# wenhao728/VORTA

Measured on AMD Instinct MI355X. Metric: video_tokens_per_sec (routed-attention denoising step, HunyuanVideo 720p 129f), higher is better.
Workload: dtype fp16

## Files before the change

### include/vorta_hip.h

```cpp
#ifndef VORTA_HIP_H
#define VORTA_HIP_H

#include <stdint.h>

#ifdef __cplusplus
extern "C" {
#endif

#define VORTA_OK 0
#define VORTA_EINVAL (-1)
#define VORTA_EUNSUPPORTED (-2)
#define VORTA_ELAUNCH (-3)

#define VORTA_ABI_VERSION 9

typedef enum vorta_dtype {
  VORTA_BF16 = 0,
  VORTA_FP16 = 1,
  VORTA_FP32 = 2,
  VORTA_FP8E4M3 = 3,
  VORTA_INT8 = 4
} vorta_dtype;

typedef struct vorta_tensor {
// ... 117 lines not shown
  float* k_bias;
  int64_t k_bias_stride_h;
  float* q_prep;
  float* k_head_scale;
  float* ws;
  int32_t flags;
  int32_t seg_len;
  int32_t tail_first;
  int32_t tail_len;
  int32_t slot_first;
  int32_t slot_count;
} vorta_i8_quant_args;

int vorta_i8_quantize_k(const vorta_i8_quant_args* args, void* hip_stream);

int vorta_i8_tail_flags(const vorta_tensor* k8, int32_t heads, int32_t n_tokens, const int32_t* row_map, float min_rms, int32_t* flags,
                        void* hip_stream);
int vorta_split_heads(const int32_t* head_list, const int32_t* n_heads_dev, int32_t n_heads, const int32_t* flags,
                      int32_t* list0, int32_t* list1, int32_t* counts, void* hip_stream);

typedef struct vorta_attn_i8_ext {
  uint32_t struct_size;
  int32_t flags;
  const float* k_bias;
  int64_t k_bias_stride_h;
  const float* q_prep;
  int64_t q_prep_stride_h;
  const float* k_head_scale;
  const float* v_descale;
  int64_t v_descale_stride_h;
// ... 141 lines not shown
```

### vorta_amd/_C.py

```python
import ctypes as C
import os

_HERE = os.path.dirname(os.path.abspath(__file__))
LIB_PATH = os.environ.get("VORTA_HIP_LIB") or os.path.join(_HERE, "csrc", "libvorta_hip.so")

VORTA_OK, VORTA_EINVAL, VORTA_EUNSUPPORTED, VORTA_ELAUNCH = 0, -1, -2, -3
VORTA_BF16, VORTA_FP16, VORTA_FP32, VORTA_FP8E4M3, VORTA_INT8 = 0, 1, 2, 3, 4
ABI_VERSION = 9

_i32, _i64, _u32, _f32, _vp = C.c_int32, C.c_int64, C.c_uint32, C.c_float, C.c_void_p


class Tensor(C.Structure):
    _fields_ = [("ptr", _vp), ("stride_h", _i64), ("stride_s", _i64)]


class AttnArgs(C.Structure):
    _fields_ = [
        ("struct_size", _u32), ("dtype", _i32), ("head_dim", _i32), ("n_heads", _i32),
        ("q", Tensor), ("k", Tensor), ("v", Tensor), ("o", Tensor),
        ("head_list", _vp), ("n_heads_dev", _vp),
        ("n_q", _i32), ("q_group_len", _i32), ("q_row_offset", _i32), ("q_valid", _i32),
        ("q_rows", _vp), ("q_rows_stride_h", _i64),
        ("n_kv", _i32), ("kv_row_offset", _i32),
# ... 136 lines not shown
NORM_ROPE_BWD_PARTS = 1024

SYMBOLS = {
    "vorta_attn_fwd": (C.c_int, [C.POINTER(AttnArgs), _vp]),
    "vorta_attn_fwd_batch": (C.c_int, [C.POINTER(AttnArgs), _i32, _vp]),
    "vorta_attn_plan": (C.c_int, [C.POINTER(AttnArgs), C.POINTER(_i32), C.POINTER(_i64), C.POINTER(_i32)]),
    "vorta_attn_workspace_bytes": (C.c_int, [C.POINTER(AttnArgs), C.POINTER(C.c_uint64), C.POINTER(C.c_uint64)]),
    "vorta_fp8_quant_ws_floats": (C.c_int, [_i32, _i32]),
    "vorta_fp8_quant_ws_partials": (C.c_int, [_i32, _i32, C.POINTER(_i64), C.POINTER(_i64)]),
    "vorta_fp8_quantize_qkv": (C.c_int, [C.POINTER(Fp8QuantArgs), _vp]),
    "vorta_fp8_v_absmax": (C.c_int, [C.POINTER(Fp8VArgs), _vp]),
    "vorta_fp8_v_convert": (C.c_int, [C.POINTER(Fp8VArgs), _vp]),
    "vorta_attn_fwd_fp8": (C.c_int, [C.POINTER(AttnArgs), C.POINTER(AttnFp8Ext), _vp]),
    "vorta_attn_fwd_batch_fp8": (C.c_int, [C.POINTER(AttnArgs), C.POINTER(AttnFp8Ext), _i32, _vp]),
    "vorta_i8_quantize_k": (C.c_int, [C.POINTER(I8QuantArgs), _vp]),
    "vorta_i8_tail_flags": (C.c_int, [C.POINTER(Tensor), _i32, _i32, _vp, C.c_float, _vp, _vp]),
    "vorta_split_heads": (C.c_int, [_vp, _vp, _i32, _vp, _vp, _vp, _vp, _vp]),
    "vorta_attn_fwd_i8": (C.c_int, [C.POINTER(AttnArgs), C.POINTER(AttnI8Ext), _vp]),
    "vorta_attn_fwd_batch_i8": (C.c_int, [C.POINTER(AttnArgs), C.POINTER(AttnI8Ext), _i32, _vp]),
    "vorta_coreset_select": (C.c_int, [C.POINTER(CoresetArgs), _vp]),
    "vorta_sta_table_sizes": (C.c_int, [C.POINTER(StaArgs), C.POINTER(_i32), C.POINTER(_i32), C.POINTER(_i32)]),
    "vorta_sta_build_tables": (C.c_int, [C.POINTER(StaArgs), _vp]),
    "vorta_router_route": (C.c_int, [C.POINTER(RouterArgs), _vp]),
    "vorta_route_scores": (C.c_int, [C.POINTER(RouterArgs), _vp]),
    "vorta_route_plan": (C.c_int, [C.POINTER(RouterArgs), C.c_int32, _vp]),
    "vorta_qk_norm_rope": (C.c_int, [C.POINTER(NormRopeArgs), _vp]),
    "vorta_qk_norm_rope_bwd": (C.c_int, [C.POINTER(NormRopeBwdArgs), _vp]),
    "vorta_mix_experts": (C.c_int, [C.POINTER(MixArgs), _vp]),
    "vorta_attn_bwd": (C.c_int, [C.POINTER(AttnBwdArgs), _vp]),
    "vorta_mix_experts_bwd": (C.c_int, [C.POINTER(MixBwdArgs), _vp]),
# ... 59 lines not shown
```

### vorta_amd/build.py

```python
import os
import subprocess
import sys

HERE = os.path.dirname(os.path.abspath(__file__))
CSRC = os.path.join(HERE, "csrc")
INCLUDE = os.path.join(os.path.dirname(HERE), "include")
LIB = os.path.join(CSRC, "libvorta_hip.so")
SOURCES = ["api.hip", "attn_fwd.hip", "attn_bwd.hip", "attn_fwd_fp8.hip", "attn_fwd_mx.hip", "attn_fwd_i8.hip", "fp8_quant.hip", "i8_quant.hip", "coreset.hip",
           "sta_tables.hip", "router.hip", "qk_norm_rope.hip", "qk_norm_rope_bwd.hip", "mix.hip", "permute.hip"]
FLAGS = ["--offload-arch=gfx950", "-O3", "-std=c++17", "-fPIC", "-fno-slp-vectorize", "-mllvm", "-enable-post-misched=0",
         "-I" + INCLUDE, "-I" + CSRC, "-Wno-unused-result"]


def _newer(src, dst):
    return (not os.path.exists(dst)) or os.path.getmtime(src) > os.path.getmtime(dst)


def build(force: bool = False, verbose: bool = True, extra_flags=None, suffix: str = "") -> str:
    hipcc = os.environ.get("HIPCC", "/opt/rocm/bin/hipcc")
    extra = list(extra_flags) if extra_flags is not None else os.environ.get("VORTA_EXTRA_FLAGS", "").split()
    suffix = suffix or os.environ.get("VORTA_BUILD_SUFFIX", "")
    if extra and not suffix:
        raise SystemExit("VORTA_EXTRA_FLAGS needs VORTA_BUILD_SUFFIX: experimental flags are never built into "
                         "libvorta_hip.so itself")
    lib = LIB if not suffix else os.path.join(CSRC, f"libvorta_hip{suffix}.so")
    deps = [os.path.join(CSRC, "common.h"), os.path.join(CSRC, "attn_common.h"), os.path.join(CSRC, "attn_fwd_fp8_diag.inc"),
            os.path.join(CSRC, "attn_fwd_i8_diag.inc"), os.path.join(CSRC, "attn_fwd_diag.inc"), os.path.join(INCLUDE, "vorta_hip.h")]
    if extra:
        extra = extra + ['-DVORTA_VARIANT_FLAGS="%s"' % " ".join(extra).replace('"', "'")]
    objs = []
    for s in SOURCES:
        src = os.path.join(CSRC, s)
        obj = os.path.join(CSRC, s.replace(".hip", f"{suffix}.o"))
        if force or _newer(src, obj) or any(_newer(d, obj) for d in deps):
            cmd = [hipcc] + FLAGS + extra + ["-c", src, "-o", obj]
            if verbose:
                print("[vorta_amd.build]", " ".join(cmd), flush=True)
            subprocess.check_call(cmd)
        objs.append(obj)
    if force or any(_newer(o, lib) for o in objs):
        cmd = [hipcc, "--offload-arch=gfx950", "-shared", "-fPIC", "-o", lib] + objs
        if verbose:
# ... 43 lines not shown
```

### vorta_amd/csrc/fp8_quant.hip

```cpp
#include <hip/hip_runtime.h>
#include <stdint.h>

#include "vorta_hip.h"
#include "common.h"

namespace {

constexpr int D = 128;
constexpr float V_TARGET = 240.f;
constexpr float E4M3_MAX = 448.f;
constexpr int MEAN_SAMPLES = 1024;
constexpr int SAMPLE_CHUNKS = 8;
constexpr int MEAN_BLOCKS = SAMPLE_CHUNKS + 1;

struct QParams {
  const char* x[3]; int64_t x_sh[3], x_ss[3];
  char* y[3]; int64_t y_sh[3], y_ss[3];
  int heads, n_tokens, rows_per_block;
  int seg_len, chunks_per_seg;
  int tail_first, tail_len;
  int mean_stride, mean_cand;
  int64_t video_tokens;
  int64_t total_tokens;
  int64_t token_offset;
  const int32_t* src_map;
// ... 201 lines not shown
  if (p.n_which < 3) return;
  float mv = p.ws[2 * H + h * D + d];
  if (p.v_per_head) {
    red[d] = mv;
    __syncthreads();
    for (int s = 64; s > 0; s >>= 1) {
      if (d < s) red[d] = fmaxf(red[d], red[d + s]);
      __syncthreads();
    }
    mv = red[0];
  }
  vmul[h * D + d] = mv > 0.f ? V_TARGET / mv : 0.f;
  p.v_descale[h * D + d] = mv / V_TARGET;
}

__device__ __forceinline__ float clamp448(float x) { return __builtin_amdgcn_fmed3f(x, -E4M3_MAX, E4M3_MAX); }

template <typename T>
__global__ __launch_bounds__(256) void fp8_convert_kernel(const QParams p) {
  typedef __attribute__((ext_vector_type(8))) T T8;
  const int which = blockIdx.z, H = p.heads;
  int r0, r1, h, hphys;
  block_rows(p, r0, r1, h, hphys);
  if (r0 >= r1) return;
  const int t = threadIdx.x, cc = t & 7, rl = t >> 3;
  const int hout = hphys;
  if (p.src_map && p.seg_len <= 0) {
    const int hs = p.src_map[hout];
    if (hs < 0) return;
    h = hphys = hs;
  }
// ... 164 lines not shown
    if (e != hipSuccess) return vorta_set_hip_error(e);
  }
  hipLaunchKernelGGL(fp8_scales_kernel, dim3((unsigned)hn), dim3(128), 0, st, p);
  e = hipGetLastError();
  if (e != hipSuccess) return vorta_set_hip_error(e);
  grid.z = (unsigned)n_which;
  if (bf) hipLaunchKernelGGL((fp8_convert_kernel<__bf16>), grid, dim3(256), 0, st, p);
  else hipLaunchKernelGGL((fp8_convert_kernel<_Float16>), grid, dim3(256), 0, st, p);
  e = hipGetLastError();
  if (e != hipSuccess) return vorta_set_hip_error(e);
  return VORTA_OK;
}

namespace {

struct VParams {
  const char* x; int64_t x_sh, x_ss;
  char* y; int64_t y_sh, y_ss;
  int heads, n_tokens, rows_per_block, per_head;
  const int32_t* src_map;
  float* amax; float* v_descale;
};

template <typename T>
__global__ __launch_bounds__(256) void fp8_v_absmax_kernel(const VParams p) {
  typedef __attribute__((ext_vector_type(8))) T T8;
  const int h = blockIdx.y;
  const int r0 = blockIdx.x * p.rows_per_block, r1 = min(r0 + p.rows_per_block, p.n_tokens);
  const int t = threadIdx.x, cc = t & 15, rl = t >> 4;
  const char* base = p.x + (int64_t)h * p.x_sh + cc * 16;
  float m[8];
#pragma unroll
  for (int i = 0; i < 8; ++i) m[i] = 0.f;
  for (int r = r0 + rl; r < r1; r += 16) {
    const T8 v = *(const T8*)(base + (int64_t)r * p.x_ss);
#pragma unroll
    for (int i = 0; i < 8; ++i) m[i] = fmaxf(m[i], fabsf(to_f(v[i])));
  }
  __shared__ float red[16][D + 1];
#pragma unroll
  for (int i = 0; i < 8; ++i) red[rl][cc * 8 + i] = m[i];
  __syncthreads();
  if (t < D) {
    float cm = 0.f;
#pragma unroll
    for (int j = 0; j < 16; ++j) cm = fmaxf(cm, red[j][t]);
    atomicMax((unsigned*)p.amax + h * D + t, __float_as_uint(cm));
  }
}

template <typename T>
__global__ __launch_bounds__(256) void fp8_v_convert_kernel(const VParams p) {
  typedef __attribute__((ext_vector_type(8))) T T8;
  const int h = blockIdx.y, hs = p.src_map ? p.src_map[h] : h;
  const int r0 = blockIdx.x * p.rows_per_block, r1 = min(r0 + p.rows_per_block, p.n_tokens);
  const int t = threadIdx.x, cc = t & 7, rl = t >> 3;
  float mul[16];
  float ph = 0.f;
  if (p.per_head) {
    for (int d = 0; d < D; ++d) ph = fmaxf(ph, p.amax[hs * D + d]);
  }
#pragma unroll
  for (int i = 0; i < 16; ++i) {
    const float mv = p.per_head ? ph : p.amax[hs * D + cc * 16 + i];
    mul[i] = mv > 0.f ? V_TARGET / mv : 0.f;
  }
  if (p.v_descale && blockIdx.x == 0 && t < D) {
    const float mv = p.per_head ? ph : p.amax[hs * D + t];
    p.v_descale[h * D + t] = mv / V_TARGET;
  }
  const char* src = p.x + (int64_t)hs * p.x_sh + cc * 32;
  char* dst = p.y + (int64_t)h * p.y_sh + cc * 16;
  for (int r = r0 + rl; r < r1; r += 32) {
    const T8 a = *(const T8*)(src + (int64_t)r * p.x_ss);
    const T8 b = *(const T8*)(src + (int64_t)r * p.x_ss + 16);
    float f[16];
#pragma unroll
    for (int i = 0; i < 8; ++i) {
      f[i] = clamp448(to_f(a[i]) * mul[i]);
      f[8 + i] = clamp448(to_f(b[i]) * mul[8 + i]);
    }
    u32x4 o;
#pragma unroll
    for (int w = 0; w < 4; ++w) {
      int lo = __builtin_amdgcn_cvt_pk_fp8_f32(f[4 * w], f[4 * w + 1], 0, false);
      o[w] = (uint32_t)__builtin_amdgcn_cvt_pk_fp8_f32(f[4 * w + 2], f[4 * w + 3], lo, true);
    }
    *(u32x4*)(dst + (int64_t)r * p.y_ss) = o;
  }
}

int v_params(const vorta_fp8_v_args* a, bool convert, VParams& p) {
  if (!a || a->struct_size != sizeof(vorta_fp8_v_args)) return VORTA_EINVAL;
  if (a->dtype != VORTA_BF16 && a->dtype != VORTA_FP16) return VORTA_EUNSUPPORTED;
  if (a->head_dim != D) return VORTA_EUNSUPPORTED;
  if (a->heads < 0 || a->n_tokens < 0) return VORTA_EINVAL;
  if (a->heads == 0 || a->n_tokens == 0) return 1;
  if (!a->amax || !a->v.ptr || ((uintptr_t)a->v.ptr & 15) || (a->v.stride_s % 8) || (a->v.stride_h % 8) || a->v.stride_s < D)
    return VORTA_EINVAL;
  p.x = (const char*)a->v.ptr; p.x_sh = a->v.stride_h * 2; p.x_ss = a->v.stride_s * 2;
  if (convert) {
    if (!a->v8.ptr || ((uintptr_t)a->v8.ptr & 15) || (a->v8.stride_s % 16) || (a->v8.stride_h % 16) || a->v8.stride_s < D)
      return VORTA_EINVAL;
    p.y = (char*)a->v8.ptr; p.y_sh = a->v8.stride_h; p.y_ss = a->v8.stride_s;
  }
  p.heads = a->heads; p.n_tokens = a->n_tokens;
  p.rows_per_block = 1024;
  p.per_head = a->flags & 1;
  p.src_map = convert ? a->src_map : nullptr;
  p.amax = a->amax; p.v_descale = convert ? a->v_descale : nullptr;
  return VORTA_OK;
}

}

extern "C" int vorta_fp8_v_absmax(const vorta_fp8_v_args* a, void* hip_stream) {
  VParams p{};
  const int rc = v_params(a, false, p);
  if (rc) return rc < 0 ? rc : VORTA_OK;
  const dim3 grid((unsigned)((p.n_tokens + p.rows_per_block - 1) / p.rows_per_block), (unsigned)p.heads);
  hipStream_t st = (hipStream_t)hip_stream;
  if (a->dtype == VORTA_BF16) hipLaunchKernelGGL((fp8_v_absmax_kernel<__bf16>), grid, dim3(256), 0, st, p);
  else hipLaunchKernelGGL((fp8_v_absmax_kernel<_Float16>), grid, dim3(256), 0, st, p);
  const hipError_t e = hipGetLastError();
  return e == hipSuccess ? VORTA_OK : vorta_set_hip_error(e);
}
// ... 13 lines not shown
```

### vorta_amd/csrc/i8_quant.hip

```cpp
#include <hip/hip_runtime.h>
#include <stdint.h>

#include "vorta_hip.h"
#include "common.h"

namespace {

constexpr int D = 128;
constexpr int SAMPLES = 1024;

struct IParams {
  const char* q; const char* k; int64_t q_sh, q_ss, k_sh, k_ss;
  char* k8; int64_t k8_sh, k8_ss;
  float* k_bias; int64_t k_bias_sh;
  float* q_prep; float* k_head_scale; float* ws;
  int heads, n_tokens, rows_per_block;
  int seg_len, chunks_per_seg, tail_first, tail_len;
  int slot_first, slot_count;
  int64_t video_tokens, total_tokens;
  int stride, cand;
  int no_smooth, no_center;
};

template <typename T>
__global__ __launch_bounds__(1024) void i8_stats_kernel(const IParams p) {
#pragma clang fp contract(off)
  typedef __attribute__((ext_vector_type(8))) T T8;
  const int h = p.slot_first + blockIdx.x;
  const int t = threadIdx.x, cg = t & 15, rl = t >> 4;
  auto row_of = [&](int64_t tok) -> int64_t {
    if (p.seg_len <= 0) return tok;
    if (tok < p.video_tokens) return ((tok / p.seg_len) * p.heads + h) * p.seg_len + tok % p.seg_len;
    return (int64_t)p.tail_first + (int64_t)h * p.seg_len + (tok - p.video_tokens);
  };
  const char* kb = p.k + (p.seg_len > 0 ? 0 : (int64_t)h * p.k_sh) + cg * 16;
  const char* qb = p.q + (p.seg_len > 0 ? 0 : (int64_t)h * p.q_sh) + cg * 16;
// ... 39 lines not shown
    const float var_k = mk2 - mean_k * mean_k;
    const float mean_q = red[2][0][t] / n;
    const float mq2 = red[3][0][t] / n;
    const float var_q = mq2 - mean_q * mean_q;
    float s = 1.f;
    if (!p.no_smooth && var_k > 0.f && var_q > 0.f) {
      s = sqrtf(sqrtf(var_k / var_q));
      s = fminf(fmaxf(s, 0.125f), 8.f);
    }
    p.ws[h * D + t] = p.no_center ? 0.f : mean_k;
    p.ws[(p.heads + h) * D + t] = 1.f / s;
    p.q_prep[(2 * h) * D + t] = p.no_center ? 0.f : mean_q;
    p.q_prep[(2 * h + 1) * D + t] = s;
  }
  if (t == 0) ((int*)p.ws)[2 * p.heads * D + h] = 0;
}

__device__ __forceinline__ void block_rows(const IParams& p, int& r0, int& r1, int& head, int& hphys) {
  if (p.seg_len > 0) {
    const int per = p.slot_count * p.chunks_per_seg;
    const int sg = blockIdx.x / per, rem = blockIdx.x - sg * per;
    const int si = rem / p.chunks_per_seg, c = rem - si * p.chunks_per_seg;
    const int seg = sg * p.heads + p.slot_first + si;
    const int s0 = seg * p.seg_len;
    r0 = s0 + c * p.rows_per_block;
    const int seg_rows = s0 >= p.tail_first ? p.tail_len : p.seg_len;
    r1 = min(min(r0 + p.rows_per_block, s0 + seg_rows), p.n_tokens);
    head = seg % p.heads;
    hphys = 0;
  } else {
    head = hphys = blockIdx.y;
    r0 = blockIdx.x * p.rows_per_block;
    r1 = min(r0 + p.rows_per_block, p.n_tokens);
  }
}

template <typename T, int PASS>
__global__ __launch_bounds__(256) void i8_rows_kernel(const IParams p) {
#pragma clang fp contract(off)
  typedef __attribute__((ext_vector_type(8))) T T8;
  int r0, r1, h, hphys;
  block_rows(p, r0, r1, h, hphys);
  if (r0 >= r1) return;
  const int t = threadIdx.x, cg = t & 15, rl = t >> 4;
  float c[8], is[8], cq[8];
#pragma unroll
  for (int e = 0; e < 8; ++e) {
    c[e] = p.ws[h * D + cg * 8 + e];
    is[e] = p.ws[(p.heads + h) * D + cg * 8 + e];
    cq[e] = p.q_prep[(2 * h) * D + cg * 8 + e];
  }
  const char* src = p.k + (int64_t)hphys * p.k_sh + cg * 16;
  char* dst = p.k8 + (int64_t)hphys * p.k8_sh + cg * 8;
  float* bias = p.k_bias + (int64_t)hphys * p.k_bias_sh;
  const float am_head = PASS == 1 ? __int_as_float(((const int*)p.ws)[2 * p.heads * D + h]) : 0.f;
  const float inv = am_head > 0.f ? 127.f / am_head : 0.f;
  float am = 0.f;
// ... 31 lines not shown
          *(u32x2*)(dst + (int64_t)r * p.k8_ss) = u32x2{w[0], w[1]};
          if (cg == 0) bias[r] = dot * inv;
        }
      }
    }
  }
  if (PASS == 0) {
    __shared__ float red[256];
    red[t] = am;
    __syncthreads();
    for (int s = 128; s > 0; s >>= 1) {
      if (t < s) red[t] = fmaxf(red[t], red[t + s]);
      __syncthreads();
    }
    if (t == 0) atomicMax((int*)p.ws + 2 * p.heads * D + h, __float_as_int(red[0]));
  }
}

__global__ void i8_head_scale_kernel(const IParams p) {
#pragma clang fp contract(off)
  const int h = p.slot_first + blockIdx.x;
  if (threadIdx.x == 0) {
    const float am = __int_as_float(((const int*)p.ws)[2 * p.heads * D + h]);
    p.k_head_scale[h] = am > 0.f ? am * (1.f / 127.f) : 1.f;
  }
}

static_assert(D == 128, "i8_tail_kernel reads a row as 8 lanes x 16 bytes and is launched with 1024 threads");
__global__ __launch_bounds__(1024) void i8_tail_kernel(const char* k8, int64_t sh, int64_t ss, const int* row_map, int n_tokens,
                                                        int stride, int cand, float min_rms, int* flags) {
// ... 56 lines not shown
                     k8->stride_s, row_map, n_tokens, stride, cand, min_rms, flags);
  const hipError_t e = hipGetLastError();
  return e == hipSuccess ? VORTA_OK : vorta_set_hip_error(e);
}

extern "C" int vorta_split_heads(const int32_t* head_list, const int32_t* n_heads_dev, int32_t n_heads, const int32_t* flags,
                                 int32_t* list0, int32_t* list1, int32_t* counts, void* hip_stream) {
  if (n_heads < 0) return VORTA_EINVAL;
  if (!flags || !list0 || !list1 || !counts) return VORTA_EINVAL;
  hipLaunchKernelGGL(split_heads_kernel, dim3(1), dim3(64), 0, (hipStream_t)hip_stream, head_list, n_heads_dev, n_heads, flags,
                     list0, list1, counts);
  const hipError_t e = hipGetLastError();
  return e == hipSuccess ? VORTA_OK : vorta_set_hip_error(e);
}

extern "C" int vorta_i8_quantize_k(const vorta_i8_quant_args* a, void* hip_stream) {
  if (!a || a->struct_size != sizeof(vorta_i8_quant_args)) return VORTA_EINVAL;
  if (a->dtype != VORTA_BF16 && a->dtype != VORTA_FP16) return VORTA_EUNSUPPORTED;
  if (a->head_dim != D) return VORTA_EUNSUPPORTED;
  if (a->heads < 0 || a->n_tokens < 0 || a->seg_len < 0 || a->tail_first < 0 || a->tail_len < 0) return VORTA_EINVAL;
  if (a->seg_len > 0 && (a->tail_first > 0 || a->tail_len > 0) && (a->tail_first % a->seg_len || a->tail_len > a->seg_len))
    return VORTA_EINVAL;
  if (a->slot_first < 0 || a->slot_count < 0 || (int64_t)a->slot_first + a->slot_count > a->heads) return VORTA_EINVAL;
  if ((a->slot_first || a->slot_count) && a->seg_len <= 0) return VORTA_EINVAL;
  if (a->heads == 0 || a->n_tokens == 0) return VORTA_OK;
  if (!a->q.ptr || !a->k.ptr || !a->k8.ptr || !a->k_bias || !a->q_prep || !a->k_head_scale || !a->ws) return VORTA_EINVAL;
  const vorta_tensor* in[2] = {&a->q, &a->k};
  for (int i = 0; i < 2; ++i)
    if (((uintptr_t)in[i]->ptr & 15) || (in[i]->stride_s % 8) || (in[i]->stride_h % 8) || in[i]->stride_s < D) return VORTA_EINVAL;
  if (((uintptr_t)a->k8.ptr & 15) || (a->k8.stride_s % 16) || (a->k8.stride_h % 16) || a->k8.stride_s < D) return VORTA_EINVAL;
  IParams p{};
  p.q = (const char*)a->q.ptr; p.k = (const char*)a->k.ptr;
  p.q_sh = a->q.stride_h * 2; p.q_ss = a->q.stride_s * 2; p.k_sh = a->k.stride_h * 2; p.k_ss = a->k.stride_s * 2;
  p.k8 = (char*)a->k8.ptr; p.k8_sh = a->k8.stride_h; p.k8_ss = a->k8.stride_s;
  p.k_bias = a->k_bias; p.k_bias_sh = a->seg_len > 0 ? 0 : a->k_bias_stride_h;
  p.q_prep = a->q_prep; p.k_head_scale = a->k_head_scale; p.ws = a->ws;
  p.heads = a->heads; p.n_tokens = a->n_tokens;
  p.seg_len = a->seg_len;
  const bool has_tail = a->seg_len > 0 && (a->tail_first > 0 || a->tail_len > 0);
  p.tail_first = has_tail ? a->tail_first : 0x7fffffff;
  p.tail_len = has_tail ? a->tail_len : 0;
  p.slot_first = a->slot_count > 0 ? a->slot_first : 0;
  p.slot_count = a->slot_count > 0 ? a->slot_count : a->heads;
  p.no_smooth = a->flags & 1; p.no_center = (a->flags >> 1) & 1;
  const int H = a->heads, hn = p.slot_count;
  int64_t head_tokens = a->n_tokens;
  p.video_tokens = head_tokens;
  if (p.seg_len > 0) {
    const int64_t data_rows = has_tail ? (int64_t)a->tail_first : (int64_t)a->n_tokens;
    p.video_tokens = (data_rows / p.seg_len / H) * p.seg_len;
    head_tokens = p.video_tokens + p.tail_len;
  }
  p.total_tokens = head_tokens;
  if (head_tokens <= 0) return VORTA_EINVAL;
  p.stride = (int)(head_tokens / SAMPLES);
  if (p.stride < 1) p.stride = 1;
  p.stride |= 1;
  p.cand = (int)((head_tokens + p.stride - 1) / p.stride);
  p.rows_per_block = 1024;
  dim3 grid;
  if (p.seg_len > 0) {
    p.chunks_per_seg = (p.seg_len + p.rows_per_block - 1) / p.rows_per_block;
    const int64_t n_seg = ((int64_t)a->n_tokens + p.seg_len - 1) / p.seg_len;
    const int64_t n_sg = (n_seg + H - 1) / H;
    if (n_sg * hn * p.chunks_per_seg > 0x7fffffffll) return VORTA_EINVAL;
    grid = dim3((unsigned)(n_sg * hn * p.chunks_per_seg), 1, 1);
  } else {
    p.chunks_per_seg = 1;
    grid = dim3((unsigned)((a->n_tokens + p.rows_per_block - 1) / p.rows_per_block), (unsigned)H, 1);
  }
  hipStream_t st = (hipStream_t)hip_stream;
  const bool bf = a->dtype == VORTA_BF16;
  if (bf) hipLaunchKernelGGL((i8_stats_kernel<__bf16>), dim3(hn), dim3(1024), 0, st, p);
  else hipLaunchKernelGGL((i8_stats_kernel<_Float16>), dim3(hn), dim3(1024), 0, st, p);
  hipError_t e = hipGetLastError();
  if (e != hipSuccess) return vorta_set_hip_error(e);
  if (bf) hipLaunchKernelGGL((i8_rows_kernel<__bf16, 0>), grid, dim3(256), 0, st, p);
  else hipLaunchKernelGGL((i8_rows_kernel<_Float16, 0>), grid, dim3(256), 0, st, p);
  e = hipGetLastError();
  if (e != hipSuccess) return vorta_set_hip_error(e);
  hipLaunchKernelGGL(i8_head_scale_kernel, dim3(hn), dim3(64), 0, st, p);
  if (bf) hipLaunchKernelGGL((i8_rows_kernel<__bf16, 1>), grid, dim3(256), 0, st, p);
  else hipLaunchKernelGGL((i8_rows_kernel<_Float16, 1>), grid, dim3(256), 0, st, p);
  e = hipGetLastError();
  if (e != hipSuccess) return vorta_set_hip_error(e);
  return VORTA_OK;
}
```

### vorta_amd/ops.py

```python
from __future__ import annotations

import ctypes as C
import math
from typing import NamedTuple, Optional, Sequence, Tuple

import torch

from . import _C

_DT = {torch.bfloat16: _C.VORTA_BF16, torch.float16: _C.VORTA_FP16}
FP8_STORAGE = torch.uint8


class Timeline:

    def __init__(self):
        self.records = []

    def summary(self):
        torch.cuda.synchronize()
        out = {}
        for tag, br, nwg, flops, e0, e1 in self.records:
            d = out.setdefault((tag, br), dict(launches=0, ms=0.0, flops=0.0, workgroups=0))
            d["launches"] += 1
# ... 405 lines not shown
class I8Operands:
    __slots__ = ("k8", "k_bias", "q_prep", "k_head_scale", "ws")

    def __init__(self, k8, k_bias, q_prep, k_head_scale, ws):
        self.k8, self.k_bias, self.q_prep, self.k_head_scale, self.ws = k8, k_bias, q_prep, k_head_scale, ws

    def k_center(self):
        H, _, D = self.q_prep.shape
        return self.ws[:H * D].view(H, D)

    def heads(self, h0: int, h1: int, k8=None, k_bias=None) -> "I8Operands":
        return I8Operands(self.k8[h0:h1] if k8 is None else k8, self.k_bias[h0:h1] if k_bias is None else k_bias,
                          self.q_prep[h0:h1], self.k_head_scale[h0:h1], self.ws)


def i8_quantize_k(q: torch.Tensor, k: torch.Tensor, *, out: Optional[I8Operands] = None, smooth: bool = True,
                  center: bool = True, heads: Optional[int] = None, seg_len: int = 0, tail_first: int = 0, tail_len: int = 0,
                  slots: Optional[Tuple[int, int]] = None) -> I8Operands:
    _require_gpu(q, k)
    if q.dtype not in _DT or q.dtype != k.dtype or q.shape != k.shape or q.dim() != 3:
        raise ValueError("i8_quantize_k takes (H,S,D) bf16 / fp16 views of q and k of equal shape")
    Hx, S, D = k.shape
    if seg_len > 0:
        if Hx != 1 or not heads or heads < 1:
            raise ValueError("i8_quantize_k: the segmented layout takes (1,rows,D) row arrays and the number of heads")
        H = heads
    else:
        if heads not in (None, Hx):
            raise ValueError("i8_quantize_k: `heads` only applies to the segmented layout")
        H = Hx
    dev = k.device
    if out is None:
        out = I8Operands(torch.empty((Hx, S, D), dtype=torch.int8, device=dev),
# ... 1 lines not shown
                         torch.empty((H, 2, D), dtype=torch.float32, device=dev),
                         torch.empty((H,), dtype=torch.float32, device=dev),
                         torch.empty(2 * H * D + H, dtype=torch.float32, device=dev))
    a = _C.I8QuantArgs()
    a.struct_size = C.sizeof(_C.I8QuantArgs)
    a.dtype, a.head_dim, a.heads, a.n_tokens = _DT[k.dtype], D, H, S
    a.q, a.k, a.k8 = _tensor(q), _tensor(k), _tensor(out.k8)
    a.k_bias, a.k_bias_stride_h = out.k_bias.data_ptr(), out.k_bias.stride(0)
    a.q_prep, a.k_head_scale, a.ws = out.q_prep.data_ptr(), out.k_head_scale.data_ptr(), out.ws.data_ptr()
    a.flags = (0 if smooth else 1) | (0 if center else 2)
    a.seg_len, a.tail_first, a.tail_len = seg_len, tail_first, tail_len
    if slots is not None:
        if seg_len <= 0 or not (0 <= slots[0] < slots[1] <= H):
            raise ValueError(f"i8_quantize_k: slots {slots} need the segmented layout and 0 <= first < end <= {H}")
        a.slot_first, a.slot_count = slots[0], slots[1] - slots[0]
    _C.check(_C.lib().vorta_i8_quantize_k(C.byref(a), _stream()), "vorta_i8_quantize_k")
    return out


I8_TAIL_MIN_RMS = float(__import__("os").environ.get("VORTA_I8_TAIL_MIN_RMS", "3.2"))


def i8_tail_flags(k8: torch.Tensor, min_rms: Optional[float] = None, out: Optional[torch.Tensor] = None,
                  row_map: Optional[torch.Tensor] = None) -> torch.Tensor:
    _require_gpu(k8)
    if k8.dtype != torch.int8 or k8.dim() != 3:
        raise ValueError("i8_tail_flags takes the (H,S,D) int8 keys of i8_quantize_k")
    H = k8.shape[0]
    n = int(row_map.numel()) if row_map is not None else k8.shape[1]
    if row_map is not None and (row_map.dtype != torch.int32 or not row_map.is_cuda or not row_map.is_contiguous()):
        raise ValueError("i8_tail_flags: row_map must be a contiguous int32 device tensor (one row of the head's view per token)")
    if out is None:
# ... 403 lines not shown
```

### vorta_amd/routed.py

```python
from __future__ import annotations

from dataclasses import dataclass, field
from typing import Dict, List, NamedTuple, Optional, Sequence, Tuple

import torch

from . import ops

Triple = Tuple[int, int, int]


@dataclass
class HeadRouting:
    lists: torch.Tensor
    counts_host: Optional[List[int]]
    counts_dev: Optional[torch.Tensor]
    partials: Optional[List[Tuple[torch.Tensor, int, int]]] = None

    @staticmethod
    def from_expert_ids(expert_of_head: Sequence[int], device, q_ranges: Optional[dict] = None) -> "HeadRouting":
        H = len(expert_of_head)
        q_ranges = q_ranges or {}
        lists = torch.zeros((3, H), dtype=torch.int32)
        counts = []
# ... 155 lines not shown
    k16: Optional[torch.Tensor] = None
    tail: Optional[torch.Tensor] = None

    def kwargs(self, scale: Optional[float]) -> dict:
        return dict(q=self.q, k=self.k, v=self.v, scale=scale, v_descale=self.v_descale, i8=self.i8)

    def tail_kwargs(self, scale: Optional[float]) -> dict:
        return dict(q=self.q, k=self.k16, v=self.v, scale=scale, v_descale=self.v_descale)


def prepare_operands(precision: str, q: torch.Tensor, k: torch.Tensor, v: torch.Tensor, scale: Optional[float],
                     fp8_operands=None, video_tokens: int = 0) -> AttnOperands:
    reuse = isinstance(fp8_operands, tuple)
    if precision in ("i8pv", "auto8"):
        vo, ko = fp8_operands if reuse and len(fp8_operands) == 2 else (None, None)
        v8, vd, _ = ops.fp8_quantize_v(v, out=vo)
        i8 = ops.i8_quantize_k(q, k, out=ko)
        tail = ops.i8_tail_flags(i8.k8) if precision == "auto8" else None
        return AttnOperands(precision, q, i8.k8, v8, vd, i8, None if tail is None else k, tail)
    if precision == "fp8pv":
        v8, vd, _ = ops.fp8_quantize_v(v, out=fp8_operands if reuse and len(fp8_operands) == 3 else None)
        return AttnOperands(precision, q, k, v8, vd)
    if precision == "fp8":
        f8 = ops.fp8_quantize_qkv(q, k, v, scale, out=fp8_operands, center_k=FP8_CENTER_K, video_tokens=video_tokens)
        return AttnOperands(precision, f8.q, f8.k, f8.v, f8.v_descale)
    return AttnOperands("native", q, k, v)


_SIDE_STREAMS: Dict[int, Tuple[torch.cuda.Stream, torch.cuda.Stream]] = {}


def _side_streams(device: torch.device):
# ... 338 lines not shown
```

### vorta_amd/ulysses/engine.py

```python
from __future__ import annotations

from typing import List, Optional, Sequence

import numpy as np
import torch
import torch.distributed as dist

from .. import ops


from .._debug import flag as _debug_flag
HIP_STAGING = _debug_flag("sp_staging", "hip") != "torch"
GROUP_STREAMS = _debug_flag("sp_group_streams", "1") != "0"
EMULATE_LINK_GBPS = float(_debug_flag("sp_emulate_link_gbps", "0") or 0)
FORCE_COLLECTIVES = __import__("os").environ.get("VORTA_SP_FORCE_COLLECTIVES", "0") == "1"
_WIRE = {}


def _wire_sleep(device, nbytes_per_link: float):
    idx = torch.device(device).index or 0
    w = _WIRE.get(idx)
    if w is None:
        st = torch.cuda.Stream(device=device)
        torch.cuda.synchronize(device)
# ... 461 lines not shown
                                  tail_first=self.rows_video, tail_len=self.T)
        shape, stride = (self.Hl, self.rows_total - (self.Hl - 1) * self.Sl, self.D), (self.Sl * self.D, self.D, 1)
        hv = lambda t: t[0].as_strided(shape, stride, t[0].storage_offset())
        vd = f8.v_descale if vwire is None else v_descale
        return hv(f8.q), hv(f8.k), hv(f8.v), vd, f8

    def i8_operands(self) -> "ops.I8Operands":
        dev = self.device
        return ops.I8Operands(torch.zeros((1, self.rows_total, self.D), dtype=torch.int8, device=dev),
                              torch.zeros((1, self.rows_total), dtype=torch.float32, device=dev),
                              torch.zeros((self.Hl, 2, self.D), dtype=torch.float32, device=dev),
                              torch.ones((self.Hl,), dtype=torch.float32, device=dev),
                              torch.zeros(2 * self.Hl * self.D + self.Hl, dtype=torch.float32, device=dev))

    def i8_views(self, bufs: Sequence[torch.Tensor], out: "ops.I8Operands"):
        ops.i8_quantize_k(bufs[0].view(1, self.rows_total, self.D), bufs[1].view(1, self.rows_total, self.D), out=out,
                          heads=self.Hl, seg_len=self.Sl, tail_first=self.rows_video, tail_len=self.T)
        rows = self.rows_total - (self.Hl - 1) * self.Sl
        k8 = out.k8[0].as_strided((self.Hl, rows, self.D), (self.Sl * self.D, self.D, 1), out.k8[0].storage_offset())
        kb = out.k_bias[0].as_strided((self.Hl, rows), (self.Sl, 1), out.k_bias[0].storage_offset())
        return ops.I8Operands(k8, kb, out.q_prep, out.k_head_scale, out.ws)

    def group_operands(self, sg: "SlotGroup", parent, cache: dict):
        if sg.lay is self:
            return parent
        key = (id(parent), sg.row0, sg.lay.Hl)
        got = cache.get(key)
        if got is None:
            n, D, dev = sg.lay.Hl, self.D, self.device
            if isinstance(parent, ops.I8Operands):
                got = ops.I8Operands(sg.buffer(parent.k8), sg.buffer(parent.k_bias), parent.q_prep[sg.g0:sg.g1],
                                     parent.k_head_scale[sg.g0:sg.g1], torch.zeros(2 * n * D + n, dtype=torch.float32, device=dev))
# ... 490 lines not shown
```

Before: 27520.

## Fuse int8 K quantization and fp8 V quantization into shared kernel launches

Result: no change. 27520 (-0.0%).

```diff
diff --git a/include/vorta_hip.h b/include/vorta_hip.h
--- a/include/vorta_hip.h
+++ b/include/vorta_hip.h
@@ -155,6 +155,8 @@
 
 int vorta_i8_quantize_k(const vorta_i8_quant_args* args, void* hip_stream);
 
+int vorta_i8pv_prepare_kv(const vorta_i8_quant_args* k_args, const vorta_fp8_v_args* v_args, void* hip_stream);
+
 int vorta_i8_tail_flags(const vorta_tensor* k8, int32_t heads, int32_t n_tokens, const int32_t* row_map, float min_rms, int32_t* flags,
                         void* hip_stream);
 int vorta_split_heads(const int32_t* head_list, const int32_t* n_heads_dev, int32_t n_heads, const int32_t* flags,
diff --git a/vorta_amd/_C.py b/vorta_amd/_C.py
--- a/vorta_amd/_C.py
+++ b/vorta_amd/_C.py
@@ -174,6 +174,7 @@
     "vorta_attn_fwd_fp8": (C.c_int, [C.POINTER(AttnArgs), C.POINTER(AttnFp8Ext), _vp]),
     "vorta_attn_fwd_batch_fp8": (C.c_int, [C.POINTER(AttnArgs), C.POINTER(AttnFp8Ext), _i32, _vp]),
     "vorta_i8_quantize_k": (C.c_int, [C.POINTER(I8QuantArgs), _vp]),
+    "vorta_i8pv_prepare_kv": (C.c_int, [C.POINTER(I8QuantArgs), C.POINTER(Fp8VArgs), _vp]),
     "vorta_i8_tail_flags": (C.c_int, [C.POINTER(Tensor), _i32, _i32, _vp, C.c_float, _vp, _vp]),
     "vorta_split_heads": (C.c_int, [_vp, _vp, _i32, _vp, _vp, _vp, _vp, _vp]),
     "vorta_attn_fwd_i8": (C.c_int, [C.POINTER(AttnArgs), C.POINTER(AttnI8Ext), _vp]),
diff --git a/vorta_amd/build.py b/vorta_amd/build.py
--- a/vorta_amd/build.py
+++ b/vorta_amd/build.py
@@ -25,7 +25,8 @@
                          "libvorta_hip.so itself")
     lib = LIB if not suffix else os.path.join(CSRC, f"libvorta_hip{suffix}.so")
     deps = [os.path.join(CSRC, "common.h"), os.path.join(CSRC, "attn_common.h"), os.path.join(CSRC, "attn_fwd_fp8_diag.inc"),
-            os.path.join(CSRC, "attn_fwd_i8_diag.inc"), os.path.join(CSRC, "attn_fwd_diag.inc"), os.path.join(INCLUDE, "vorta_hip.h")]
+            os.path.join(CSRC, "attn_fwd_i8_diag.inc"), os.path.join(CSRC, "attn_fwd_diag.inc"), os.path.join(CSRC, "fp8_v_rows.h"),
+            os.path.join(INCLUDE, "vorta_hip.h")]
     if extra:
         extra = extra + ['-DVORTA_VARIANT_FLAGS="%s"' % " ".join(extra).replace('"', "'")]
     objs = []
diff --git a/vorta_amd/csrc/fp8_quant.hip b/vorta_amd/csrc/fp8_quant.hip
--- a/vorta_amd/csrc/fp8_quant.hip
+++ b/vorta_amd/csrc/fp8_quant.hip
@@ -3,12 +3,11 @@
 
 #include "vorta_hip.h"
 #include "common.h"
+#include "fp8_v_rows.h"
 
 namespace {
 
 constexpr int D = 128;
-constexpr float V_TARGET = 240.f;
-constexpr float E4M3_MAX = 448.f;
 constexpr int MEAN_SAMPLES = 1024;
 constexpr int SAMPLE_CHUNKS = 8;
 constexpr int MEAN_BLOCKS = SAMPLE_CHUNKS + 1;
@@ -240,7 +239,6 @@
   p.v_descale[h * D + d] = mv / V_TARGET;
 }
 
-__device__ __forceinline__ float clamp448(float x) { return __builtin_amdgcn_fmed3f(x, -E4M3_MAX, E4M3_MAX); }
 
 template <typename T>
 __global__ __launch_bounds__(256) void fp8_convert_kernel(const QParams p) {
@@ -435,102 +433,14 @@
 
 namespace {
 
-struct VParams {
-  const char* x; int64_t x_sh, x_ss;
-  char* y; int64_t y_sh, y_ss;
-  int heads, n_tokens, rows_per_block, per_head;
-  const int32_t* src_map;
-  float* amax; float* v_descale;
-};
-
 template <typename T>
 __global__ __launch_bounds__(256) void fp8_v_absmax_kernel(const VParams p) {
-  typedef __attribute__((ext_vector_type(8))) T T8;
-  const int h = blockIdx.y;
-  const int r0 = blockIdx.x * p.rows_per_block, r1 = min(r0 + p.rows_per_block, p.n_tokens);
-  const int t = threadIdx.x, cc = t & 15, rl = t >> 4;
-  const char* base = p.x + (int64_t)h * p.x_sh + cc * 16;
-  float m[8];
-#pragma unroll
-  for (int i = 0; i < 8; ++i) m[i] = 0.f;
-  for (int r = r0 + rl; r < r1; r += 16) {
-    const T8 v = *(const T8*)(base + (int64_t)r * p.x_ss);
-#pragma unroll
-    for (int i = 0; i < 8; ++i) m[i] = fmaxf(m[i], fabsf(to_f(v[i])));
-  }
-  __shared__ float red[16][D + 1];
-#pragma unroll
-  for (int i = 0; i < 8; ++i) red[rl][cc * 8 + i] = m[i];
-  __syncthreads();
-  if (t < D) {
-    float cm = 0.f;
-#pragma unroll
-    for (int j = 0; j < 16; ++j) cm = fmaxf(cm, red[j][t]);
-    atomicMax((unsigned*)p.amax + h * D + t, __float_as_uint(cm));
-  }
+  v_absmax_rows<T>(p, blockIdx.y, blockIdx.x);
 }
 
 template <typename T>
 __global__ __launch_bounds__(256) void fp8_v_convert_kernel(const VParams p) {
-  typedef __attribute__((ext_vector_type(8))) T T8;
-  const int h = blockIdx.y, hs = p.src_map ? p.src_map[h] : h;
-  const int r0 = blockIdx.x * p.rows_per_block, r1 = min(r0 + p.rows_per_block, p.n_tokens);
-  const int t = threadIdx.x, cc = t & 7, rl = t >> 3;
-  float mul[16];
-  float ph = 0.f;
-  if (p.per_head) {
-    for (int d = 0; d < D; ++d) ph = fmaxf(ph, p.amax[hs * D + d]);
-  }
-#pragma unroll
-  for (int i = 0; i < 16; ++i) {
-    const float mv = p.per_head ? ph : p.amax[hs * D + cc * 16 + i];
-    mul[i] = mv > 0.f ? V_TARGET / mv : 0.f;
-  }
-  if (p.v_descale && blockIdx.x == 0 && t < D) {
-    const float mv = p.per_head ? ph : p.amax[hs * D + t];
-    p.v_descale[h * D + t] = mv / V_TARGET;
-  }
-  const char* src = p.x + (int64_t)hs * p.x_sh + cc * 32;
-  char* dst = p.y + (int64_t)h * p.y_sh + cc * 16;
-  for (int r = r0 + rl; r < r1; r += 32) {
-    const T8 a = *(const T8*)(src + (int64_t)r * p.x_ss);
-    const T8 b = *(const T8*)(src + (int64_t)r * p.x_ss + 16);
-    float f[16];
-#pragma unroll
-    for (int i = 0; i < 8; ++i) {
-      f[i] = clamp448(to_f(a[i]) * mul[i]);
-      f[8 + i] = clamp448(to_f(b[i]) * mul[8 + i]);
-    }
-    u32x4 o;
-#pragma unroll
-    for (int w = 0; w < 4; ++w) {
-      int lo = __builtin_amdgcn_cvt_pk_fp8_f32(f[4 * w], f[4 * w + 1], 0, false);
-      o[w] = (uint32_t)__builtin_amdgcn_cvt_pk_fp8_f32(f[4 * w + 2], f[4 * w + 3], lo, true);
-    }
-    *(u32x4*)(dst + (int64_t)r * p.y_ss) = o;
-  }
-}
-
-int v_params(const vorta_fp8_v_args* a, bool convert, VParams& p) {
-  if (!a || a->struct_size != sizeof(vorta_fp8_v_args)) return VORTA_EINVAL;
-  if (a->dtype != VORTA_BF16 && a->dtype != VORTA_FP16) return VORTA_EUNSUPPORTED;
-  if (a->head_dim != D) return VORTA_EUNSUPPORTED;
-  if (a->heads < 0 || a->n_tokens < 0) return VORTA_EINVAL;
-  if (a->heads == 0 || a->n_tokens == 0) return 1;
-  if (!a->amax || !a->v.ptr || ((uintptr_t)a->v.ptr & 15) || (a->v.stride_s % 8) || (a->v.stride_h % 8) || a->v.stride_s < D)
-    return VORTA_EINVAL;
-  p.x = (const char*)a->v.ptr; p.x_sh = a->v.stride_h * 2; p.x_ss = a->v.stride_s * 2;
-  if (convert) {
-    if (!a->v8.ptr || ((uintptr_t)a->v8.ptr & 15) || (a->v8.stride_s % 16) || (a->v8.stride_h % 16) || a->v8.stride_s < D)
-      return VORTA_EINVAL;
-    p.y = (char*)a->v8.ptr; p.y_sh = a->v8.stride_h; p.y_ss = a->v8.stride_s;
-  }
-  p.heads = a->heads; p.n_tokens = a->n_tokens;
-  p.rows_per_block = 1024;
-  p.per_head = a->flags & 1;
-  p.src_map = convert ? a->src_map : nullptr;
-  p.amax = a->amax; p.v_descale = convert ? a->v_descale : nullptr;
-  return VORTA_OK;
+  v_convert_rows<T>(p, blockIdx.y, blockIdx.x);
 }
 
 }
diff --git a/vorta_amd/csrc/fp8_v_rows.h b/vorta_amd/csrc/fp8_v_rows.h
--- /dev/null
+++ b/vorta_amd/csrc/fp8_v_rows.h
@@ -0,0 +1,113 @@
+#pragma once
+#include <hip/hip_runtime.h>
+#include <stdint.h>
+
+#include "vorta_hip.h"
+#include "common.h"
+
+namespace {
+
+constexpr int V_D = 128;
+constexpr float V_TARGET = 240.f;
+constexpr float E4M3_MAX = 448.f;
+
+__device__ __forceinline__ float clamp448(float x) { return __builtin_amdgcn_fmed3f(x, -E4M3_MAX, E4M3_MAX); }
+
+struct VParams {
+  const char* x; int64_t x_sh, x_ss;
+  char* y; int64_t y_sh, y_ss;
+  int heads, n_tokens, rows_per_block, per_head;
+  const int32_t* src_map;
+  float* amax; float* v_descale;
+};
+
+template <typename T>
+__device__ __forceinline__ void v_absmax_rows(const VParams& p, int h, int chunk) {
+  typedef __attribute__((ext_vector_type(8))) T T8;
+  const int r0 = chunk * p.rows_per_block, r1 = min(r0 + p.rows_per_block, p.n_tokens);
+  const int t = threadIdx.x, cc = t & 15, rl = t >> 4;
+  const char* base = p.x + (int64_t)h * p.x_sh + cc * 16;
+  float m[8];
+#pragma unroll
+  for (int i = 0; i < 8; ++i) m[i] = 0.f;
+  for (int r = r0 + rl; r < r1; r += 16) {
+    const T8 v = *(const T8*)(base + (int64_t)r * p.x_ss);
+#pragma unroll
+    for (int i = 0; i < 8; ++i) m[i] = fmaxf(m[i], fabsf((float)v[i]));
+  }
+  __shared__ float red[16][V_D + 1];
+#pragma unroll
+  for (int i = 0; i < 8; ++i) red[rl][cc * 8 + i] = m[i];
+  __syncthreads();
+  if (t < V_D) {
+    float cm = 0.f;
+#pragma unroll
+    for (int j = 0; j < 16; ++j) cm = fmaxf(cm, red[j][t]);
+    atomicMax((unsigned*)p.amax + h * V_D + t, __float_as_uint(cm));
+  }
+}
+
+template <typename T>
+__device__ __forceinline__ void v_convert_rows(const VParams& p, int h, int chunk) {
+  typedef __attribute__((ext_vector_type(8))) T T8;
+  const int hs = p.src_map ? p.src_map[h] : h;
+  const int r0 = chunk * p.rows_per_block, r1 = min(r0 + p.rows_per_block, p.n_tokens);
+  const int t = threadIdx.x, cc = t & 7, rl = t >> 3;
+  float mul[16];
+  float ph = 0.f;
+  if (p.per_head) {
+    for (int d = 0; d < V_D; ++d) ph = fmaxf(ph, p.amax[hs * V_D + d]);
+  }
+#pragma unroll
+  for (int i = 0; i < 16; ++i) {
+    const float mv = p.per_head ? ph : p.amax[hs * V_D + cc * 16 + i];
+    mul[i] = mv > 0.f ? V_TARGET / mv : 0.f;
+  }
+  if (p.v_descale && chunk == 0 && t < V_D) {
+    const float mv = p.per_head ? ph : p.amax[hs * V_D + t];
+    p.v_descale[h * V_D + t] = mv / V_TARGET;
+  }
+  const char* src = p.x + (int64_t)hs * p.x_sh + cc * 32;
+  char* dst = p.y + (int64_t)h * p.y_sh + cc * 16;
+  for (int r = r0 + rl; r < r1; r += 32) {
+    const T8 a = *(const T8*)(src + (int64_t)r * p.x_ss);
+    const T8 b = *(const T8*)(src + (int64_t)r * p.x_ss + 16);
+    float f[16];
+#pragma unroll
+    for (int i = 0; i < 8; ++i) {
+      f[i] = clamp448((float)a[i] * mul[i]);
+      f[8 + i] = clamp448((float)b[i] * mul[8 + i]);
+    }
+    u32x4 o;
+#pragma unroll
+    for (int w = 0; w < 4; ++w) {
+      int lo = __builtin_amdgcn_cvt_pk_fp8_f32(f[4 * w], f[4 * w + 1], 0, false);
+      o[w] = (uint32_t)__builtin_amdgcn_cvt_pk_fp8_f32(f[4 * w + 2], f[4 * w + 3], lo, true);
+    }
+    *(u32x4*)(dst + (int64_t)r * p.y_ss) = o;
+  }
+}
+
+inline int v_params(const vorta_fp8_v_args* a, bool convert, VParams& p) {
+  if (!a || a->struct_size != sizeof(vorta_fp8_v_args)) return VORTA_EINVAL;
+  if (a->dtype != VORTA_BF16 && a->dtype != VORTA_FP16) return VORTA_EUNSUPPORTED;
+  if (a->head_dim != V_D) return VORTA_EUNSUPPORTED;
+  if (a->heads < 0 || a->n_tokens < 0) return VORTA_EINVAL;
+  if (a->heads == 0 || a->n_tokens == 0) return 1;
+  if (!a->amax || !a->v.ptr || ((uintptr_t)a->v.ptr & 15) || (a->v.stride_s % 8) || (a->v.stride_h % 8) || a->v.stride_s < V_D)
+    return VORTA_EINVAL;
+  p.x = (const char*)a->v.ptr; p.x_sh = a->v.stride_h * 2; p.x_ss = a->v.stride_s * 2;
+  if (convert) {
+    if (!a->v8.ptr || ((uintptr_t)a->v8.ptr & 15) || (a->v8.stride_s % 16) || (a->v8.stride_h % 16) || a->v8.stride_s < V_D)
+      return VORTA_EINVAL;
+    p.y = (char*)a->v8.ptr; p.y_sh = a->v8.stride_h; p.y_ss = a->v8.stride_s;
+  }
+  p.heads = a->heads; p.n_tokens = a->n_tokens;
+  p.rows_per_block = 1024;
+  p.per_head = a->flags & 1;
+  p.src_map = convert ? a->src_map : nullptr;
+  p.amax = a->amax; p.v_descale = convert ? a->v_descale : nullptr;
+  return VORTA_OK;
+}
+
+}
diff --git a/vorta_amd/csrc/i8_quant.hip b/vorta_amd/csrc/i8_quant.hip
--- a/vorta_amd/csrc/i8_quant.hip
+++ b/vorta_amd/csrc/i8_quant.hip
@@ -3,6 +3,7 @@
 
 #include "vorta_hip.h"
 #include "common.h"
+#include "fp8_v_rows.h"
 
 namespace {
 
@@ -20,6 +21,7 @@
   int64_t video_tokens, total_tokens;
   int stride, cand;
   int no_smooth, no_center;
+  float* v_amax; int v_amax_n;
 };
 
 template <typename T>
@@ -89,12 +91,13 @@
     p.q_prep[(2 * h + 1) * D + t] = s;
   }
   if (t == 0) ((int*)p.ws)[2 * p.heads * D + h] = 0;
-}
-
-__device__ __forceinline__ void block_rows(const IParams& p, int& r0, int& r1, int& head, int& hphys) {
+  for (int i = blockIdx.x * 1024 + t; i < p.v_amax_n; i += gridDim.x * 1024) p.v_amax[i] = 0.f;
+}
+
+__device__ __forceinline__ void block_rows(const IParams& p, int bx, int by, int& r0, int& r1, int& head, int& hphys, bool& first) {
   if (p.seg_len > 0) {
     const int per = p.slot_count * p.chunks_per_seg;
-    const int sg = blockIdx.x / per, rem = blockIdx.x - sg * per;
+    const int sg = bx / per, rem = bx - sg * per;
     const int si = rem / p.chunks_per_seg, c = rem - si * p.chunks_per_seg;
     const int seg = sg * p.heads + p.slot_first + si;
     const int s0 = seg * p.seg_len;
@@ -103,19 +106,26 @@
     r1 = min(min(r0 + p.rows_per_block, s0 + seg_rows), p.n_tokens);
     head = seg % p.heads;
     hphys = 0;
+    first = sg == 0 && c == 0;
   } else {
-    head = hphys = blockIdx.y;
-    r0 = blockIdx.x * p.rows_per_block;
+    head = hphys = by;
+    r0 = bx * p.rows_per_block;
     r1 = min(r0 + p.rows_per_block, p.n_tokens);
-  }
-}
-
-template <typename T, int PASS>
-__global__ __launch_bounds__(256) void i8_rows_kernel(const IParams p) {
+    first = bx == 0;
+  }
+}
+
+template <typename T, int PASS, bool SCALE>
+__device__ __forceinline__ void i8_rows(const IParams& p, int bx, int by) {
 #pragma clang fp contract(off)
   typedef __attribute__((ext_vector_type(8))) T T8;
   int r0, r1, h, hphys;
-  block_rows(p, r0, r1, h, hphys);
+  bool first;
+  block_rows(p, bx, by, r0, r1, h, hphys, first);
+  if (SCALE && first && threadIdx.x == 0) {
+    const float am = __int_as_float(((const int*)p.ws)[2 * p.heads * D + h]);
+    p.k_head_scale[h] = am > 0.f ? am * (1.f / 127.f) : 1.f;
+  }
   if (r0 >= r1) return;
   const int t = threadIdx.x, cg = t & 15, rl = t >> 4;
   float c[8], is[8], cq[8];
@@ -177,6 +187,30 @@
       __syncthreads();
     }
     if (t == 0) atomicMax((int*)p.ws + 2 * p.heads * D + h, __float_as_int(red[0]));
+  }
+}
+
+template <typename T, int PASS>
+__global__ __launch_bounds__(256) void i8_rows_kernel(const IParams p) {
+  i8_rows<T, PASS, false>(p, blockIdx.x, blockIdx.y);
+}
+
+struct KVParams {
+  IParams k;
+  VParams v;
+  int k_blocks, k_gx, v_gx;
+};
+
+template <typename T, int PASS>
+__global__ __launch_bounds__(256) void i8pv_kv_kernel(const KVParams p) {
+  const int b = blockIdx.x;
+  if (b < p.k_blocks) {
+    const int by = b / p.k_gx;
+    i8_rows<T, PASS, PASS == 1>(p.k, b - by * p.k_gx, by);
+  } else {
+    const int vb = b - p.k_blocks, h = vb / p.v_gx;
+    if (PASS == 0) v_absmax_rows<T>(p.v, h, vb - h * p.v_gx);
+    else v_convert_rows<T>(p.v, h, vb - h * p.v_gx);
   }
 }
 
@@ -263,7 +297,9 @@
   return e == hipSuccess ? VORTA_OK : vorta_set_hip_error(e);
 }
 
-extern "C" int vorta_i8_quantize_k(const vorta_i8_quant_args* a, void* hip_stream) {
+namespace {
+
+int k_params(const vorta_i8_quant_args* a, IParams& p, dim3& grid) {
   if (!a || a->struct_size != sizeof(vorta_i8_quant_args)) return VORTA_EINVAL;
   if (a->dtype != VORTA_BF16 && a->dtype != VORTA_FP16) return VORTA_EUNSUPPORTED;
   if (a->head_dim != D) return VORTA_EUNSUPPORTED;
@@ -272,13 +308,12 @@
     return VORTA_EINVAL;
   if (a->slot_first < 0 || a->slot_count < 0 || (int64_t)a->slot_first + a->slot_count > a->heads) return VORTA_EINVAL;
   if ((a->slot_first || a->slot_count) && a->seg_len <= 0) return VORTA_EINVAL;
-  if (a->heads == 0 || a->n_tokens == 0) return VORTA_OK;
+  if (a->heads == 0 || a->n_tokens == 0) return 1;
   if (!a->q.ptr || !a->k.ptr || !a->k8.ptr || !a->k_bias || !a->q_prep || !a->k_head_scale || !a->ws) return VORTA_EINVAL;
   const vorta_tensor* in[2] = {&a->q, &a->k};
   for (int i = 0; i < 2; ++i)
     if (((uintptr_t)in[i]->ptr & 15) || (in[i]->stride_s % 8) || (in[i]->stride_h % 8) || in[i]->stride_s < D) return VORTA_EINVAL;
   if (((uintptr_t)a->k8.ptr & 15) || (a->k8.stride_s % 16) || (a->k8.stride_h % 16) || a->k8.stride_s < D) return VORTA_EINVAL;
-  IParams p{};
   p.q = (const char*)a->q.ptr; p.k = (const char*)a->k.ptr;
   p.q_sh = a->q.stride_h * 2; p.q_ss = a->q.stride_s * 2; p.k_sh = a->k.stride_h * 2; p.k_ss = a->k.stride_s * 2;
   p.k8 = (char*)a->k8.ptr; p.k8_sh = a->k8.stride_h; p.k8_ss = a->k8.stride_s;
@@ -307,7 +342,6 @@
   p.stride |= 1;
   p.cand = (int)((head_tokens + p.stride - 1) / p.stride);
   p.rows_per_block = 1024;
-  dim3 grid;
   if (p.seg_len > 0) {
     p.chunks_per_seg = (p.seg_len + p.rows_per_block - 1) / p.rows_per_block;
     const int64_t n_seg = ((int64_t)a->n_tokens + p.seg_len - 1) / p.seg_len;
@@ -318,6 +352,17 @@
     p.chunks_per_seg = 1;
     grid = dim3((unsigned)((a->n_tokens + p.rows_per_block - 1) / p.rows_per_block), (unsigned)H, 1);
   }
+  return VORTA_OK;
+}
+
+}
+
+extern "C" int vorta_i8_quantize_k(const vorta_i8_quant_args* a, void* hip_stream) {
+  IParams p{};
+  dim3 grid;
+  const int rc = k_params(a, p, grid);
+  if (rc) return rc < 0 ? rc : VORTA_OK;
+  const int hn = p.slot_count;
   hipStream_t st = (hipStream_t)hip_stream;
   const bool bf = a->dtype == VORTA_BF16;
   if (bf) hipLaunchKernelGGL((i8_stats_kernel<__bf16>), dim3(hn), dim3(1024), 0, st, p);
@@ -335,3 +380,45 @@
   if (e != hipSuccess) return vorta_set_hip_error(e);
   return VORTA_OK;
 }
+
+extern "C" int vorta_i8pv_prepare_kv(const vorta_i8_quant_args* ka, const vorta_fp8_v_args* va, void* hip_stream) {
+  KVParams p{};
+  dim3 kgrid;
+  const int rk = k_params(ka, p.k, kgrid);
+  if (rk < 0) return rk;
+  int rv = 1;
+  if (va) {
+    rv = v_params(va, true, p.v);
+    if (rv < 0) return rv;
+    if (va->src_map) return VORTA_EUNSUPPORTED;
+    if (!rk && va->dtype != ka->dtype) return VORTA_EINVAL;
+  }
+  if (rk && rv) return VORTA_OK;
+  const int64_t k_blocks = rk ? 0 : (int64_t)kgrid.x * kgrid.y;
+  p.k_gx = rk ? 1 : (int)kgrid.x;
+  p.v_gx = rv ? 1 : (p.v.n_tokens + p.v.rows_per_block - 1) / p.v.rows_per_block;
+  const int64_t blocks = k_blocks + (rv ? 0 : (int64_t)p.v_gx * p.v.heads);
+  if (blocks > 0x7fffffffll) return VORTA_EINVAL;
+  p.k_blocks = (int)k_blocks;
+  hipStream_t st = (hipStream_t)hip_stream;
+  const bool bf = (rk ? va->dtype : ka->dtype) == VORTA_BF16;
+  hipError_t e;
+  if (!rk) {
+    if (!rv) { p.k.v_amax = p.v.amax; p.k.v_amax_n = p.v.heads * V_D; }
+    if (bf) hipLaunchKernelGGL((i8_stats_kernel<__bf16>), dim3(p.k.slot_count), dim3(1024), 0, st, p.k);
+    else hipLaunchKernelGGL((i8_stats_kernel<_Float16>), dim3(p.k.slot_count), dim3(1024), 0, st, p.k);
+    e = hipGetLastError();
+  } else {
+    e = hipMemsetAsync(p.v.amax, 0, sizeof(float) * p.v.heads * V_D, st);
+  }
+  if (e != hipSuccess) return vorta_set_hip_error(e);
+  if (bf) hipLaunchKernelGGL((i8pv_kv_kernel<__bf16, 0>), dim3((unsigned)blocks), dim3(256), 0, st, p);
+  else hipLaunchKernelGGL((i8pv_kv_kernel<_Float16, 0>), dim3((unsigned)blocks), dim3(256), 0, st, p);
+  e = hipGetLastError();
+  if (e != hipSuccess) return vorta_set_hip_error(e);
+  if (bf) hipLaunchKernelGGL((i8pv_kv_kernel<__bf16, 1>), dim3((unsigned)blocks), dim3(256), 0, st, p);
+  else hipLaunchKernelGGL((i8pv_kv_kernel<_Float16, 1>), dim3((unsigned)blocks), dim3(256), 0, st, p);
+  e = hipGetLastError();
+  if (e != hipSuccess) return vorta_set_hip_error(e);
+  return VORTA_OK;
+}
diff --git a/vorta_amd/ops.py b/vorta_amd/ops.py
--- a/vorta_amd/ops.py
+++ b/vorta_amd/ops.py
@@ -443,9 +443,7 @@
                           self.q_prep[h0:h1], self.k_head_scale[h0:h1], self.ws)
 
 
-def i8_quantize_k(q: torch.Tensor, k: torch.Tensor, *, out: Optional[I8Operands] = None, smooth: bool = True,
-                  center: bool = True, heads: Optional[int] = None, seg_len: int = 0, tail_first: int = 0, tail_len: int = 0,
-                  slots: Optional[Tuple[int, int]] = None) -> I8Operands:
+def _i8_quant_args(q, k, out, smooth, center, heads, seg_len, tail_first, tail_len, slots):
     _require_gpu(q, k)
     if q.dtype not in _DT or q.dtype != k.dtype or q.shape != k.shape or q.dim() != 3:
         raise ValueError("i8_quantize_k takes (H,S,D) bf16 / fp16 views of q and k of equal shape")
@@ -477,8 +475,44 @@
         if seg_len <= 0 or not (0 <= slots[0] < slots[1] <= H):
             raise ValueError(f"i8_quantize_k: slots {slots} need the segmented layout and 0 <= first < end <= {H}")
         a.slot_first, a.slot_count = slots[0], slots[1] - slots[0]
+    return a, out
+
+
+def i8_quantize_k(q: torch.Tensor, k: torch.Tensor, *, out: Optional[I8Operands] = None, smooth: bool = True,
+                  center: bool = True, heads: Optional[int] = None, seg_len: int = 0, tail_first: int = 0, tail_len: int = 0,
+                  slots: Optional[Tuple[int, int]] = None) -> I8Operands:
+    a, out = _i8_quant_args(q, k, out, smooth, center, heads, seg_len, tail_first, tail_len, slots)
     _C.check(_C.lib().vorta_i8_quantize_k(C.byref(a), _stream()), "vorta_i8_quantize_k")
     return out
+
+
+def i8pv_prepare_kv(q: torch.Tensor, k: torch.Tensor, v: Optional[torch.Tensor], *, out=None, smooth: bool = True,
+                    center: bool = True, heads: Optional[int] = None, seg_len: int = 0, tail_first: int = 0,
+                    tail_len: int = 0, slots: Optional[Tuple[int, int]] = None):
+    vo, ko = out if out is not None else (None, None)
+    a, ko = _i8_quant_args(q, k, ko, smooth, center, heads, seg_len, tail_first, tail_len, slots)
+    va = None
+    if v is not None:
+        if v.dtype != k.dtype:
+            raise ValueError("i8pv_prepare_kv: k and v must share their dtype")
+        if vo is None:
+            Hv, Sv, D = v.shape
+            vo = (torch.empty((Hv, Sv, D), dtype=FP8_STORAGE, device=v.device),
+                  torch.empty((Hv, D), dtype=torch.float32, device=v.device),
+                  torch.empty((Hv, D), dtype=torch.float32, device=v.device))
+        v8, vd, amax = vo
+        if amax.shape[0] != v.shape[0]:
+            raise ValueError("i8pv_prepare_kv: amax needs one row per head of v")
+        va = _fp8_v_args(v, amax, False)
+        _require_gpu(v8, vd)
+        if v8.dtype != FP8_STORAGE or v8.shape != v.shape:
+            raise ValueError("i8pv_prepare_kv: v8 must be a uint8 view with v's shape")
+        if vd.dtype != torch.float32 or not vd.is_contiguous() or tuple(vd.shape) != (v.shape[0], v.shape[2]):
+            raise ValueError("i8pv_prepare_kv: v_descale must be a contiguous float32 (heads of v, D) tensor")
+        va.v8, va.v_descale = _tensor(v8), vd.data_ptr()
+    _C.check(_C.lib().vorta_i8pv_prepare_kv(C.byref(a), C.byref(va) if va is not None else None, _stream()),
+             "vorta_i8pv_prepare_kv")
+    return (vo if v is not None else None), ko
 
 
 I8_TAIL_MIN_RMS = float(__import__("os").environ.get("VORTA_I8_TAIL_MIN_RMS", "3.2"))
diff --git a/vorta_amd/routed.py b/vorta_amd/routed.py
--- a/vorta_amd/routed.py
+++ b/vorta_amd/routed.py
@@ -193,8 +193,7 @@
     reuse = isinstance(fp8_operands, tuple)
     if precision in ("i8pv", "auto8"):
         vo, ko = fp8_operands if reuse and len(fp8_operands) == 2 else (None, None)
-        v8, vd, _ = ops.fp8_quantize_v(v, out=vo)
-        i8 = ops.i8_quantize_k(q, k, out=ko)
+        (v8, vd, _), i8 = ops.i8pv_prepare_kv(q, k, v, out=(vo, ko))
         tail = ops.i8_tail_flags(i8.k8) if precision == "auto8" else None
         return AttnOperands(precision, q, i8.k8, v8, vd, i8, None if tail is None else k, tail)
     if precision == "fp8pv":
diff --git a/vorta_amd/ulysses/engine.py b/vorta_amd/ulysses/engine.py
--- a/vorta_amd/ulysses/engine.py
+++ b/vorta_amd/ulysses/engine.py
@@ -499,8 +499,8 @@
                               torch.zeros(2 * self.Hl * self.D + self.Hl, dtype=torch.float32, device=dev))
 
     def i8_views(self, bufs: Sequence[torch.Tensor], out: "ops.I8Operands"):
-        ops.i8_quantize_k(bufs[0].view(1, self.rows_total, self.D), bufs[1].view(1, self.rows_total, self.D), out=out,
-                          heads=self.Hl, seg_len=self.Sl, tail_first=self.rows_video, tail_len=self.T)
+        ops.i8pv_prepare_kv(bufs[0].view(1, self.rows_total, self.D), bufs[1].view(1, self.rows_total, self.D), None,
+                            out=(None, out), heads=self.Hl, seg_len=self.Sl, tail_first=self.rows_video, tail_len=self.T)
         rows = self.rows_total - (self.Hl - 1) * self.Sl
         k8 = out.k8[0].as_strided((self.Hl, rows, self.D), (self.Sl * self.D, self.D, 1), out.k8[0].storage_offset())
         kb = out.k_bias[0].as_strided((self.Hl, rows), (self.Sl, 1), out.k_bias[0].storage_offset())
```
